# Dellintel98/smart-nanogrid-gym

Measured on AMD Instinct MI355X. Metric: env-steps/sec (whole node) at N=65,536 envs × 10 chargers, 24-step day, higher is better.
Workload: dtype f64; 1 GPU; 65536 envs/GPU x 10 chargers x 24-step day, b-pv bounded sparse 1h, GPU-RNG reset + 24 fused steps per bench step (hipGraph); envs_per_gpu=65536, chargers=10, step_unit=one simulated day of every env, days_per_graph_replay=11, parallelism=env-sharded x1

## Files before the change

smart-nanogrid-gym_amd/csrc/sng_generate.h:

```cpp
#pragma once

namespace sng {

struct HashStream {
    uint32_t key, ctr;
    __device__ __forceinline__ uint32_t next() { return mix32(key + (ctr++) * 0x9e3779b9u); }
};

__device__ __forceinline__ double u32_unit(uint32_t x) { return (double)x * 0x1.0p-32; }

__device__ __forceinline__ int below(uint32_t x, int n) {
    return (int)(((uint64_t)x * (uint64_t)n) >> 32);
}

constexpr uint32_t kDomainRatio = 0x7a710000u;
constexpr uint32_t kDomainReplay = 0x7a720000u;

__device__ __forceinline__ double pv_ratio_draw(uint64_t seed, uint64_t ge, uint64_t day) {
    HashStream r2{stream_key(seed, ge, kDomainRatio, day), 0u};
    return (double)below(r2.next(), 181) / 100;
}

__device__ __forceinline__ double replay_ratio_draw(uint64_t seed, uint64_t ge, uint64_t replay) {
    HashStream r2{stream_key(seed, ge, kDomainReplay, replay), 0u};
    return (double)below(r2.next(), 181) / 100;
}

__device__ __noinline__ void mt_twist_lane(const uint32_t *A, uint32_t *B);
__device__ __forceinline__ double py_ratio_lane(const RefStreams &ps, int64_t e, bool end_draw, bool draw,
                                                double keep) {
    uint32_t *blk = ps.mt + (size_t)e * 2 * kMtN;
    const int32_t pos = ps.pos[e];
    int cur = (pos >> 16) & 1, mti = pos & kMtPosMask;
    bool ready = (pos & kMtNextReady) != 0;
    auto next = [&]() -> uint32_t {
        if (mti >= kMtN) {
            if (!ready) mt_twist_lane(blk + cur * kMtN, blk + (cur ^ 1) * kMtN);
            cur ^= 1;
            mti -= kMtN;
            ready = false;
        }
        return blk[cur * kMtN + mti++];
    };
    auto randint180 = [&]() -> int {
        uint32_t r;
        do {
            r = next() >> 24;
        } while (r >= 181u);
        return (int)r;
    };
    if (end_draw) (void)randint180();
    const double ratio = draw ? (double)randint180() / 100 : keep;
    ps.pos[e] = (cur << 16) | (ready ? kMtNextReady : 0) | mti;
    return ratio;
}

template <int BLOCK, bool PK>
__global__ __launch_bounds__(BLOCK) void observe0_kernel(Params p, DeviceState s, float *__restrict__ obs,
                                                         double *__restrict__ ep_return, int64_t E, int vec_io,
                                                         int mode, int64_t replay, RefStreams ps, int py) {
    extern __shared__ __attribute__((aligned(16))) float lds[];
    const int n = p.n, O = p.obs_dim;
    const int tid = threadIdx.x;
    const int64_t e0 = (int64_t)blockIdx.x * BLOCK;
    const int nblk = (int)((E - e0) < BLOCK ? (E - e0) : BLOCK);
    const int64_t e = e0 + tid;
    float *o_row = lds + tid * O;
    if (tid < nblk) {
        const uint64_t ge = (uint64_t)(e + p.env_offset);
        double ratio;
        if (py) {
            ratio = py_ratio_lane(ps, e, (py & 2) != 0, (py & 1) != 0, 0.0);
            if (py & 1)
                s.ratio[e] = ratio;
            else
                ratio = s.ratio[e];
        } else if (mode == OBS0_DEVICE) {
            ratio = pv_ratio_draw(p.seed, ge, *s.episode);
            s.ratio[e] = ratio;
        } else if (mode == OBS0_REPLAY && replay >= 0) {
            ratio = replay_ratio_draw(p.seed, ge, (uint64_t)replay);
            s.ratio[e] = ratio;
        } else {
            ratio = s.ratio[e];
        }
        if (mode != OBS0_HOST) s.pen0[e] = 0.0;
        double fpv[4] = {1.0, 1.0, 1.0, 1.0}, fpr[4] = {1.0, 1.0, 1.0, 1.0};
        if (p.noise) profile_factors(p, s, (uint32_t)e * 8u, 0, fpv, fpr);
        write_obs_header(o_row, p, s.tables->irr_norm, s.tables->price_norm, ratio, fpv, fpr);
        const int k = p.pv ? 8 : 4;
        const uint32_t *__restrict__ word = s.word;
        const double *__restrict__ auxv = s.aux;
        double *__restrict__ socv = s.soc;
        constexpr int B = 16;
        for (int c0 = 0; c0 < n; c0 += B) {
            uint32_t w[B];
            double aux[B];
            if (PK) {
                const uint16_t *rec = packed_records(s);
                uint32_t r0[B], r1[B];
#pragma unroll
                for (int j = 0; j < B; ++j) {
                    const int c = c0 + j < n ? c0 + j : n - 1;
                    const size_t ri = rec_index(c, e, n, E);
                    r1[j] = rec[(size_t)n * E + ri];
                    r0[j] = rec[ri];
                }
#pragma unroll
                for (int j = 0; j < B; ++j) {
                    w[j] = (r1[j] & W_OCC) ? r1[j] : 0u;
                    aux[j] = (r1[j] & W_OCC) ? (double)rec_soc(r0[j]) : 0.0;
                }
            } else {
#pragma unroll
                for (int j = 0; j < B; ++j) {
                    const int c = c0 + j < n ? c0 + j : n - 1;
                    w[j] = word[(size_t)c * E + e];
                    aux[j] = auxv[(size_t)c * E + e];
                }
            }
#pragma unroll
            for (int j = 0; j < B; ++j) {
                const int c = c0 + j;
                if (c < n) {
                    if (c + 1 < n && !(j & 1))
                        bst2<kNT>(socv, (uint32_t)soc_index(c, e, n, E) * 8u, aux[j], aux[j + 1 < B ? j + 1 : j]);
                    else if (c + 1 == n && !(j & 1))
                        bst<kNT>(socv, (uint32_t)soc_index(c, e, n, E) * 8u, aux[j]);
                    o_row[k + c] = (float)aux[j];
                    o_row[k + n + c] = departure_obs<PK>(w[j]);
                }
            }
        }
        if (p.bess) o_row[O - 1] = (float)s.bess[e];
        if (ep_return) ep_return[e] = 0.0;
    }
    if ((mode == OBS0_HOST || mode == OBS0_GENERATED) && blockIdx.x == 0 && tid == 0) *s.episode += 1;
    __syncthreads();
    copy_out<BLOCK>(obs + e0 * O, lds, nblk * O, vec_io != 0, tid);
}

__global__ __launch_bounds__(256) void profile_kernel(Params p, DeviceState s, int64_t E) {
    const int64_t e = (int64_t)blockIdx.x * 256 + threadIdx.x;
    if (e >= E) return;
    const uint64_t day = *s.episode;
    const uint64_t env_seed = p.seed + (uint64_t)p.env_offset + (uint64_t)e;
    s.prof_key[2 * e] = stream_key(env_seed, 0, kDomainPV, day);
    s.prof_key[2 * e + 1] = stream_key(env_seed, 0, kDomainPrice, day);
}


constexpr int kGenBlock = 256;
constexpr int kDayVehicles = 8;
constexpr float kInvLog2Q = -1.3569154488567239f;

constexpr int kDaySlots = kDayVehicles + 1;
__host__ __device__ constexpr size_t generate_lds_bytes(bool with_req) {
    return (size_t)kDaySlots * kGenBlock * (sizeof(uint32_t) + sizeof(float) + (with_req ? sizeof(double) : 0));
}

struct VehicleDraw {
    int ta, dep;
    uint32_t cap;
    double soc;
    uint32_t req_draw;
    uint32_t code;
};
__device__ __forceinline__ uint32_t mix32_gen(uint32_t x) {
    x ^= x >> 16;
    x *= 0x7feb352du;
    x ^= x >> 15;
    x *= 0x846ca68bu;
    x ^= x >> 16;
    return x;
}
struct GenStream {
    uint32_t key, ctr;
    __device__ __forceinline__ uint32_t next() { return mix32_gen(key + (ctr++) * 0x9e3779b9u); }
};
__device__ __forceinline__ uint32_t gen_key(uint64_t seed, uint64_t ge, uint32_t c, uint64_t day) {
    const uint32_t k0 = mix32((uint32_t)seed ^ mix32((uint32_t)(seed >> 32) + (uint32_t)day * 0x9e3779b9u));
    return mix32((k0 + (uint32_t)(ge >> 25) * 0x85ebca6bu) ^ (((uint32_t)ge << 7) | c));
}
__device__ __forceinline__ VehicleDraw draw_vehicle(const Params &p, GenStream &rng, int tfree, int i4, int i10,
                                                    int i1) {
    VehicleDraw d;
    const uint32_t x1 = rng.next(), x2 = rng.next();
    const float u = ((float)(x1 >> 8) + 1.0f) * 0x1.0p-24f;
    d.ta = tfree + (int)(__log2f(u) * kInvLog2Q);
    d.code = x2 >> (32 - kSocCodeBits);
    d.soc = (double)code_soc(d.code);
    const uint32_t r = ((x1 & 0xffu) << 8) | (x2 & 0xffu);
    const uint32_t rc = r * 105u;
    d.cap = p.diff_caps ? 15u + (rc >> 16) : 40u;
    const uint32_t yd = (p.diff_caps ? rc : r) & 0xffffu;
    const int hi_c = d.ta + i10, hi_d = p.T + i1;
    const int high = hi_c < hi_d ? hi_c : hi_d;
    const int low = d.ta + i4;
    d.dep = (low >= high) ? low : low + (int)(__umul24(yd, (uint32_t)(high - low)) >> 16);
    d.req_draw = p.req_enabled ? rng.next() : 0u;
    return d;
}

constexpr int kObsParts = kGenBlock / kWave;
constexpr int kObsEnvs = kGenBlock / kObsParts;
constexpr int kObsBlocks = kGenBlock / kObsEnvs;
static_assert(kObsEnvs == kGenObsEnvs, "generator_fused (sng_graph_form.h) sizes the observation tile");
__device__ __forceinline__ void observe_day0(const Params &p, const DeviceState &s, uint64_t seed, int64_t E, int i4,
                                             int i10, int i1, uint64_t day, float *__restrict__ obs,
                                             double *__restrict__ ep_return, int vec_io, float *lds, int q) {
    const int n = p.n, O = p.obs_dim;
    const int tid = threadIdx.x, part = __builtin_amdgcn_readfirstlane(tid / kWave), le = tid % kWave;
    const int64_t e0 = (int64_t)blockIdx.x * kGenBlock + (int64_t)q * kObsEnvs;
    if (e0 >= E) return;
    const int nblk = (int)((E - e0) < kObsEnvs ? (E - e0) : kObsEnvs);
    const int64_t e = e0 + le;
    float *o_row = lds + le * O;
    if (le < nblk) {
        const uint64_t ge = (uint64_t)(e + p.env_offset);
        const uint64_t env_seed = p.seed + (uint64_t)p.env_offset + (uint64_t)e;
        if (p.noise && part == 0) {
            s.prof_key[2 * e] = stream_key(env_seed, 0, kDomainPV, day);
            s.prof_key[2 * e + 1] = stream_key(env_seed, 0, kDomainPrice, day);
        }
        if (part == 0) {
            const double ratio = pv_ratio_draw(seed, ge, day);
            s.ratio[e] = ratio;
            s.pen0[e] = 0.0;
            double fpv[4] = {1.0, 1.0, 1.0, 1.0}, fpr[4] = {1.0, 1.0, 1.0, 1.0};
            if (p.noise) {
#pragma unroll
                for (int k = 0; k < 4; ++k) {
                    if (p.pv_noise != 0.0) fpv[k] = profile_factor(env_seed, kDomainPV, day, k, p.pv_noise);
                    if (p.price_noise != 0.0) fpr[k] = profile_factor(env_seed, kDomainPrice, day, k, p.price_noise);
                }
            }
            if (obs) {
                write_obs_header(o_row, p, s.tables->irr_norm, s.tables->price_norm, ratio, fpv, fpr);
                if (p.bess) o_row[O - 1] = (float)s.bess[e];
            }
            if (ep_return) ep_return[e] = 0.0;
        }
        const int k = p.pv ? 8 : 4;
        const uint32_t el8 = (uint32_t)e * 8u;
        for (int c0 = 2 * (part - 1); part > 0 && c0 < n; c0 += 2 * (kObsParts - 1)) {
            double soc0[2] = {0.0, 0.0};
#pragma unroll
            for (int i = 0; i < 2; ++i) {
                const int c = c0 + i;
                if (c >= n) break;
                GenStream rng{gen_key(seed, ge, (uint32_t)c, day), 0u};
                const VehicleDraw d = draw_vehicle(p, rng, 0, i4, i10, i1);
                const bool occ0 = d.ta == 0;
                soc0[i] = occ0 ? d.soc : 0.0;
                if (obs) {
                    o_row[k + c] = (float)soc0[i];
                    o_row[k + n + c] = departure_obs(pack_word(occ0, occ0, false, 0u, occ0 ? (uint32_t)d.dep : 0u));
                }
            }
            const SocOff so = soc_off(c0, n, E, el8);
            if (c0 + 1 < n)
                bst2<kNT>(s.soc, so.v, soc0[0], soc0[1], so.s);
            else
                bst<kNT>(s.soc, so.v, soc0[0], so.s);
        }
    }
    if (!obs) return;
    __syncthreads();
    copy_out<kGenBlock>(obs + e0 * O, lds, nblk * O, vec_io != 0, tid);
}

constexpr int kGenRecPol = kNT;
__host__ __device__ constexpr int gen_part_lanes(int w) { return w == 3 ? 4 : w; }
__host__ __device__ constexpr int gen_rows(int n) { return 4 * (n / 4) + (n % 4 == 0 ? 0 : 4 * gen_part_lanes(n % 4) / 4); }
constexpr int kVehArrShift = 24;
constexpr uint32_t kVehRecMask = 0x3fff8u;
template <int TT, bool REQ>
__global__ __launch_bounds__(kGenBlock) void generate_kernel(Params p, DeviceState s, uint64_t seed, int64_t E,
                                                             int i4, int i10, int i1, float *__restrict__ obs,
                                                             double *__restrict__ ep_return, int vec_io,
                                                             int day_delta) {
    extern __shared__ __attribute__((aligned(16))) float lds[];
    uint32_t *s_veh = reinterpret_cast<uint32_t *>(lds);
    uint32_t *s_car = s_veh + kDaySlots * kGenBlock;
    double *s_req = reinterpret_cast<double *>(s_car + kDaySlots * kGenBlock);
    const int tid = threadIdx.x;
    const int u = (int)blockIdx.y;
    const uint64_t day = *s.episode + (uint64_t)day_delta;
    if (u >= gen_rows(p.n)) {
        observe_day0(p, s, seed, E, i4, i10, i1, day, obs, ep_return, vec_io, lds, u - gen_rows(p.n));
        return;
    }
    const int full = 4 * (p.n / 4);
    const int q4 = u < full ? (u >> 2) * 4 : p.n & ~3;
    const int qw = p.n - q4 < 4 ? p.n - q4 : 4;
    const int lpe = u < full ? 4 : gen_part_lanes(qw);
    const int sub = u < full ? (u & 3) : u - full;
    const int c = q4 + tid % lpe;
    const int64_t e = (int64_t)blockIdx.x * kGenBlock + (int64_t)sub * (kGenBlock / lpe) + tid / lpe;
    if (e >= E || c >= p.n) return;
    const uint64_t ge = (uint64_t)(e + p.env_offset);
    GenStream rng{gen_key(seed, ge, (uint32_t)c, day), 0u};
    const int T = TT > 0 ? TT : p.T;
    const int n = p.n;

    int tfree = 0, nv = 0;
    for (int v = 0; v < kDayVehicles - 1; ++v) {
        if (tfree >= T) break;
        const VehicleDraw d = draw_vehicle(p, rng, tfree, i4, i10, i1);
        if (d.ta >= T) break;
        s_veh[v * kGenBlock + tid] = ((uint32_t)d.ta << kVehArrShift) | (d.cap << P_CAP_SHIFT) | ((uint32_t)d.dep << P_DEP_SHIFT);
        s_car[v * kGenBlock + tid] = rec_carry(false, d.code);
        if (REQ) {
            const double lo = d.soc <= 0.9 ? d.soc + 0.1 : 1.0;
            s_req[v * kGenBlock + tid] = lo + (1.0 - lo) * u32_unit(d.req_draw);
        }
        nv = v + 1;
        tfree = d.dep + 1;
    }

    s_veh[nv * kGenBlock + tid] = (0xffu << kVehArrShift) | (0xffu << P_DEP_SHIFT);
    s_car[nv * kGenBlock + tid] = 0u;
    if (REQ) s_req[nv * kGenBlock + tid] = 1.0;

    uint32_t cur = s_veh[tid], nxt = s_veh[kGenBlock + tid];
    uint32_t car_cur = s_car[tid], car_nxt = s_car[kGenBlock + tid];
    double req_cur = REQ ? s_req[tid] : 1.0, req_nxt = REQ ? s_req[kGenBlock + tid] : 1.0;
    int nx = kGenBlock + tid;
    bool prev_occ = false;
    bool pen = false;
    bool occ = (cur >> kVehArrShift) == 0u, stat = occ;
    const uint32_t pen_lo = (p.penalty_mode == SNG_PENALTY_NONE) ? 256u : 1u;
    const uint32_t pen_span = (p.penalty_mode == SNG_PENALTY_SPARSE) ? 2u
                              : (p.penalty_mode == SNG_PENALTY_DENSE) ? 254u : 0u;
    const uint32_t el2 = ((uint32_t)e * (uint32_t)qw + (uint32_t)(c - q4)) * 2u;
    const uint32_t r2 = (uint32_t)q4 * (uint32_t)E * 2u;
    const uint32_t el8 = ((uint32_t)c * (uint32_t)E + (uint32_t)e) * 8u;
    uint16_t *rec = reinterpret_cast<uint16_t *>(s.aux);
    const size_t nE = (size_t)n * (size_t)E;
    bst16<kGenRecPol>(rec, el2, ((cur >> kVehArrShift) == 0u) ? car_cur : 0u, r2);
#pragma unroll
    for (int t = 0; t < T; ++t) {
        const bool adv = (uint32_t)(t + 1) > ((cur >> P_DEP_SHIFT) & 0xffu);
        const uint32_t v1 = adv ? nxt : cur;
        const uint32_t car1 = adv ? car_nxt : car_cur;
        const double req1 = adv ? req_nxt : req_cur;
        nx += adv ? kGenBlock : 0;
        const uint32_t nxt1 = s_veh[nx];
        const uint32_t car_nxt1 = s_car[nx];
        const double req_nxt1 = REQ ? s_req[nx] : 1.0;

        const uint32_t flags = W_OCC | (stat ? W_STATIC : 0u) | (pen ? W_PEN : 0u);
        const uint32_t w_occ = ((cur & kVehRecMask) | flags) - ((uint32_t)t << P_DEP_SHIFT);
        const bool arr1 = (v1 >> kVehArrShift) == (uint32_t)(t + 1);
        const uint32_t carry = arr1 ? car1 : 0u;
        const uint32_t w_emp = (pen ? W_PEN : 0u) | carry;
        bst16<kGenRecPol>(rec + (size_t)(t + 1) * nE, el2, occ ? w_occ : w_emp, r2);
        if (REQ && t > 0) bst(s.req + (size_t)t * nE, el8, prev_occ ? req_cur : 0.0);
        prev_occ = occ;
        pen = occ && (w_occ >> P_DEP_SHIFT) - pen_lo <= pen_span;
        occ = (occ && (uint32_t)(t + 1) < ((cur >> P_DEP_SHIFT) & 0xffu)) || arr1;
        stat = arr1;
        cur = v1;
        car_cur = car1;
        req_cur = req1;
        nxt = nxt1;
        car_nxt = car_nxt1;
        req_nxt = req_nxt1;
    }
    if (REQ) bst(s.req, el8, prev_occ ? req_cur : 0.0);
}

}
```

Before: 20.78 billion env-steps/s.

## Restructure generator day loop with pre-encoded occupancy bits and simplified penalty logic

Vehicle records are pre-tagged with the occupancy flag and an arrival bit in the carry word, so the per-timestep loop derives occupancy, static and penalty flags with fewer compares and shifts. The penalty test becomes a single threshold compare, the LDS pointer is advanced directly, and the trailing req store is folded into the loop. When no observation buffer is requested, the generator threads write initial SOC themselves and the observe-day0 parts other than 0 exit early. The cap/yd computation drops a branch by using a single 24-bit multiply. The penalty threshold remap and the bit-packing shift are easy to get wrong and could change outputs.

```diff
diff --git a/smart-nanogrid-gym_amd/csrc/sng_generate.h b/smart-nanogrid-gym_amd/csrc/sng_generate.h
--- a/smart-nanogrid-gym_amd/csrc/sng_generate.h
+++ b/smart-nanogrid-gym_amd/csrc/sng_generate.h
@@ -191,9 +191,9 @@
     d.code = x2 >> (32 - kSocCodeBits);
     d.soc = (double)code_soc(d.code);
     const uint32_t r = ((x1 & 0xffu) << 8) | (x2 & 0xffu);
-    const uint32_t rc = r * 105u;
-    d.cap = p.diff_caps ? 15u + (rc >> 16) : 40u;
-    const uint32_t yd = (p.diff_caps ? rc : r) & 0xffffu;
+    const uint32_t rc = __umul24(r, p.diff_caps ? 105u : 1u);
+    d.cap = (p.diff_caps ? 15u : 40u) + (rc >> 16);
+    const uint32_t yd = rc & 0xffffu;
     const int hi_c = d.ta + i10, hi_d = p.T + i1;
     const int high = hi_c < hi_d ? hi_c : hi_d;
     const int low = d.ta + i4;
@@ -213,6 +213,7 @@
     const int tid = threadIdx.x, part = __builtin_amdgcn_readfirstlane(tid / kWave), le = tid % kWave;
     const int64_t e0 = (int64_t)blockIdx.x * kGenBlock + (int64_t)q * kObsEnvs;
     if (e0 >= E) return;
+    if (!obs && part > 0) return;
     const int nblk = (int)((E - e0) < kObsEnvs ? (E - e0) : kObsEnvs);
     const int64_t e = e0 + le;
     float *o_row = lds + le * O;
@@ -274,7 +275,7 @@
 __host__ __device__ constexpr int gen_part_lanes(int w) { return w == 3 ? 4 : w; }
 __host__ __device__ constexpr int gen_rows(int n) { return 4 * (n / 4) + (n % 4 == 0 ? 0 : 4 * gen_part_lanes(n % 4) / 4); }
 constexpr int kVehArrShift = 24;
-constexpr uint32_t kVehRecMask = 0x3fff8u;
+constexpr int kCarArrBit = 17;
 template <int TT, bool REQ>
 __global__ __launch_bounds__(kGenBlock) void generate_kernel(Params p, DeviceState s, uint64_t seed, int64_t E,
                                                              int i4, int i10, int i1, float *__restrict__ obs,
@@ -309,8 +310,9 @@
         if (tfree >= T) break;
         const VehicleDraw d = draw_vehicle(p, rng, tfree, i4, i10, i1);
         if (d.ta >= T) break;
-        s_veh[v * kGenBlock + tid] = ((uint32_t)d.ta << kVehArrShift) | (d.cap << P_CAP_SHIFT) | ((uint32_t)d.dep << P_DEP_SHIFT);
-        s_car[v * kGenBlock + tid] = rec_carry(false, d.code);
+        s_veh[v * kGenBlock + tid] =
+            ((uint32_t)d.ta << kVehArrShift) | (d.cap << P_CAP_SHIFT) | ((uint32_t)d.dep << P_DEP_SHIFT) | W_OCC;
+        s_car[v * kGenBlock + tid] = rec_carry(false, d.code) | (1u << kCarArrBit);
         if (REQ) {
             const double lo = d.soc <= 0.9 ? d.soc + 0.1 : 1.0;
             s_req[v * kGenBlock + tid] = lo + (1.0 - lo) * u32_unit(d.req_draw);
@@ -326,41 +328,45 @@
     uint32_t cur = s_veh[tid], nxt = s_veh[kGenBlock + tid];
     uint32_t car_cur = s_car[tid], car_nxt = s_car[kGenBlock + tid];
     double req_cur = REQ ? s_req[tid] : 1.0, req_nxt = REQ ? s_req[kGenBlock + tid] : 1.0;
-    int nx = kGenBlock + tid;
-    bool prev_occ = false;
-    bool pen = false;
-    bool occ = (cur >> kVehArrShift) == 0u, stat = occ;
-    const uint32_t pen_lo = (p.penalty_mode == SNG_PENALTY_NONE) ? 256u : 1u;
-    const uint32_t pen_span = (p.penalty_mode == SNG_PENALTY_SPARSE) ? 2u
-                              : (p.penalty_mode == SNG_PENALTY_DENSE) ? 254u : 0u;
+    const uint32_t *pn = s_veh + kGenBlock + tid;
+    bool occ = cur < (1u << kVehArrShift);
+    uint32_t stat_bit = occ ? W_STATIC : 0u, pen_bit = 0u;
+    const uint32_t pen_hi = p.penalty_mode == SNG_PENALTY_NONE     ? 0u
+                            : p.penalty_mode == SNG_PENALTY_SPARSE ? 4u << P_DEP_SHIFT
+                            : p.penalty_mode == SNG_PENALTY_DENSE  ? 0xffffu
+                                                                   : 2u << P_DEP_SHIFT;
     const uint32_t el2 = ((uint32_t)e * (uint32_t)qw + (uint32_t)(c - q4)) * 2u;
     const uint32_t r2 = (uint32_t)q4 * (uint32_t)E * 2u;
     const uint32_t el8 = ((uint32_t)c * (uint32_t)E + (uint32_t)e) * 8u;
+    const size_t nE = (size_t)n * (size_t)E;
     uint16_t *rec = reinterpret_cast<uint16_t *>(s.aux);
-    const size_t nE = (size_t)n * (size_t)E;
-    bst16<kGenRecPol>(rec, el2, ((cur >> kVehArrShift) == 0u) ? car_cur : 0u, r2);
+    bst16<kGenRecPol>(rec, el2, occ ? car_cur : 0u, r2);
+    if (!obs) {
+        const SocOff so = soc_off(c, n, E, (uint32_t)e * 8u);
+        bst<kNT>(s.soc, so.v + so.s, occ ? (double)rec_soc(car_cur) : 0.0);
+    }
 #pragma unroll
     for (int t = 0; t < T; ++t) {
-        const bool adv = (uint32_t)(t + 1) > ((cur >> P_DEP_SHIFT) & 0xffu);
+        const uint32_t w_occ = cur - ((uint32_t)t << P_DEP_SHIFT);
+        const uint32_t left16 = w_occ & 0xffffu;
+        const bool adv = occ && left16 < (2u << P_DEP_SHIFT);
+        const bool pen1 = occ && left16 < pen_hi;
         const uint32_t v1 = adv ? nxt : cur;
         const uint32_t car1 = adv ? car_nxt : car_cur;
         const double req1 = adv ? req_nxt : req_cur;
-        nx += adv ? kGenBlock : 0;
-        const uint32_t nxt1 = s_veh[nx];
-        const uint32_t car_nxt1 = s_car[nx];
-        const double req_nxt1 = REQ ? s_req[nx] : 1.0;
-
-        const uint32_t flags = W_OCC | (stat ? W_STATIC : 0u) | (pen ? W_PEN : 0u);
-        const uint32_t w_occ = ((cur & kVehRecMask) | flags) - ((uint32_t)t << P_DEP_SHIFT);
-        const bool arr1 = (v1 >> kVehArrShift) == (uint32_t)(t + 1);
-        const uint32_t carry = arr1 ? car1 : 0u;
-        const uint32_t w_emp = (pen ? W_PEN : 0u) | carry;
-        bst16<kGenRecPol>(rec + (size_t)(t + 1) * nE, el2, occ ? w_occ : w_emp, r2);
-        if (REQ && t > 0) bst(s.req + (size_t)t * nE, el8, prev_occ ? req_cur : 0.0);
-        prev_occ = occ;
-        pen = occ && (w_occ >> P_DEP_SHIFT) - pen_lo <= pen_span;
-        occ = (occ && (uint32_t)(t + 1) < ((cur >> P_DEP_SHIFT) & 0xffu)) || arr1;
-        stat = arr1;
+        pn += adv ? kGenBlock : 0;
+        const uint32_t nxt1 = pn[0];
+        const uint32_t car_nxt1 = pn[kDaySlots * kGenBlock];
+        const double req_nxt1 = REQ ? s_req[pn - s_veh] : 1.0;
+
+        const bool occ1 = v1 < ((uint32_t)(t + 2) << kVehArrShift);
+        const uint32_t w = occ ? w_occ : occ1 ? car1 : 0u;
+        rec += nE;
+        bst16<kGenRecPol>(rec, el2, w | stat_bit | pen_bit, r2);
+        if (REQ) bst(s.req + (size_t)(t + 1 < T ? t + 1 : 0) * nE, el8, occ ? req_cur : 0.0);
+        stat_bit = (w >> (kCarArrBit - 1)) & W_STATIC;
+        pen_bit = pen1 ? W_PEN : 0u;
+        occ = occ1;
         cur = v1;
         car_cur = car1;
         req_cur = req1;
@@ -368,7 +374,6 @@
         car_nxt = car_nxt1;
         req_nxt = req_nxt1;
     }
-    if (REQ) bst(s.req, el8, prev_occ ? req_cur : 0.0);
-}
-
-}
+}
+
+}
```

New measurement: 20.94 billion env-steps/s, median of 5. Within noise of the previous version (+0.8%).
